# QuakeMigrate/QuakeMigrate

Measured on AMD Instinct MI355X. Metric: grid-nodes x time-samples stacked /sec (detect sweep), higher is better.
Workload: dtype f64

## Files before the change

### __graft_entry__.py

```python

import pathlib
import shutil
import subprocess
import sys
import sysconfig

ROOT = pathlib.Path(__file__).resolve().parent
CSRC = ROOT / "quakemigrate_amd" / "csrc"
if str(ROOT) not in sys.path:
    sys.path.insert(0, str(ROOT))

HIPCC_FLAGS = ["--offload-arch=gfx950", "-O3", "-std=c++17", "-fPIC"]
OBJ = CSRC / "build"


def _run(cmd, **kw):
    print("+", " ".join(str(c) for c in cmd), flush=True)
    subprocess.check_call([str(c) for c in cmd], **kw)


def _stale(target, sources):
    if not target.exists():
        return True
    t = target.stat().st_mtime
    return any(pathlib.Path(s).stat().st_mtime > t for s in sources)


def build_engine(force=False):
    import concurrent.futures
    import os

    for generator, include in (("gen_ring_asm.py", "qm_ring_asm.inc"), ("gen_shift_asm.py", "qm_shift_asm.inc")):
        gen = subprocess.check_output([sys.executable, str(CSRC / generator)], text=True)
        inc = CSRC / include
        if not inc.exists() or inc.read_text() != gen:
            inc.write_text(gen)
    srcs = sorted(CSRC.glob("qm_*.hip")) + [CSRC / "qm_stalta.cpp"]
    headers = sorted(CSRC.glob("*.hpp")) + sorted(CSRC.glob("*.inc")) + [ROOT / "include" / "qmhip.h"]
    link_inputs = [CSRC / "qmhip.map"]
    hipcc = shutil.which("hipcc") or "/opt/rocm/bin/hipcc"
    OBJ.mkdir(exist_ok=True)
    objs = [OBJ / (src.name + ".o") for src in srcs]
    lib = CSRC / "libqmhip.so"
    todo = []
    if force or _stale(lib, srcs + headers):
        todo = [(src, obj) for src, obj in zip(srcs, objs) if force or _stale(obj, [src] + headers)]
    if todo:
        todo.sort(key=lambda so: ("pair" not in so[0].name, "exact" not in so[0].name))
        with concurrent.futures.ThreadPoolExecutor(max(1, min(len(todo), os.cpu_count() or 1))) as pool:
            asm_unit = ["-Wno-inline-asm", "-Wno-pass-failed", "-save-temps=obj", "-Wno-unused-command-line-argument"]
            quiet = {"qm_launch_shift.hip": asm_unit, "qm_launch_shift_sets.hip": asm_unit}
            list(pool.map(lambda so: _run([hipcc, *HIPCC_FLAGS, *quiet.get(so[0].name, []), "-c", so[0],
                                           "-o", so[1]]), todo))
        if any(src.name.startswith("qm_launch_shift") for src, _ in todo):
            check_row_block_registers()
    if force or todo or _stale(lib, srcs + headers + link_inputs):
        _run([hipcc, "--offload-arch=gfx950", "-shared", "-fPIC", f"-Wl,--version-script={CSRC / 'qmhip.map'}",
              "-o", lib, *objs])
    alias = CSRC / ("qmlib" + sysconfig.get_config_var("EXT_SUFFIX"))
    if force or _stale(alias, [lib]):
        shutil.copyfile(lib, alias)
    return lib


def check_row_block_registers():
    sys.path.insert(0, str(CSRC))
    try:
        import check_shift_isa
    finally:
        sys.path.pop(0)
    found = sorted(OBJ.glob("qm_launch_shift-*gfx950*.s"))
    if not found:
        raise RuntimeError("build: the ISA of qm_launch_shift.hip was not kept (-save-temps=obj): the "
                           "row-block kernels' register convention cannot be checked")
    n = check_shift_isa.check_all(found[-1].read_text(), (CSRC / "qm_shift_asm.inc").read_text())
    print(f"build: row-block kernels keep to their registers ({n} compiler instructions checked)")
    for tmp in OBJ.glob("qm_launch_shift*"):
        if tmp.suffix in (".bc", ".hipi", ".hipfb", ".out", ".o", ".txt") and not tmp.name.endswith(".hip.o"):
            tmp.unlink()
        elif tmp.suffix == ".s" and "gfx950" not in tmp.name:
            tmp.unlink()


def build_oracle():
    _run(["make", "-C", ROOT / "oracle", "libqm_oracle.so"])
    _run(["make", "-C", ROOT / "oracle", "ref"])


def build():
    build_engine()
    build_oracle()
    import quakemigrate_amd
    from quakemigrate_amd import core

    print("build ok:", CSRC / "libqmhip.so")


def smoke():
    import numpy as np

    from oracle import qm_oracle
    from quakemigrate_amd import synth
    from quakemigrate_amd.core import lib

    if lib.qmlib.qm_device_count() < 1:
        raise RuntimeError("smoke(): no HIP device visible")
    case = synth.make_case("C2", step=0, grid=(26, 25, 14), n_samples=700)
    a, b, c = lib.migrate_and_find_max(case.onsets, case.traveltimes, case.fsmp,
                                       case.lsmp, case.available)
    ra, rb, rc = qm_oracle.detect(case.onsets, case.traveltimes, case.fsmp,
                                  case.lsmp, case.available, threads=4)
    assert np.array_equal(c, rc), "argmax mismatch vs oracle"
    np.testing.assert_allclose(a, ra, rtol=1e-6)
    np.testing.assert_allclose(b, rb, rtol=1e-6)
    print("smoke ok: fused detect == oracle on", case.grid, "x", case.n_samples,
          "samples; max rel err", float(np.max(np.abs(a - ra) / ra)))


if __name__ == "__main__":
    build()
    if len(sys.argv) > 1 and sys.argv[1] == "smoke":
        smoke()
```

### quakemigrate_amd/csrc/qm_shift.hpp

```cpp
#pragma once

#include "qm_kernels.hpp"

namespace qm {

struct ShiftStageNext {
    const void *meta;
    int rows;
    int first_row, stride;
    const void *src;
    unsigned row_bytes;
    unsigned lds;
    unsigned lane32;
};

#ifndef QM_SHIFT_ASM_INC
#define QM_SHIFT_ASM_INC "qm_shift_asm.inc"
#endif
#include QM_SHIFT_ASM_INC

constexpr int kShiftWaves = 4;
constexpr int kShiftWaves8 = 8;
constexpr int kShiftWaves3 = 12;
constexpr int kShiftKT = 256;
constexpr int kShiftWideKT = kWave * kShiftWideSpl;
constexpr int kShiftLdsBytes = 2 * kShiftPlane;
constexpr int kShiftStateBytes = 5 * kShiftStateChunk;
constexpr int kShiftLdsBytes3 = 2 * kShiftPlane3 + kShiftWaves3 * kShiftStateBytes;
static_assert(kShiftLdsBytes3 <= 160 * 1024, "the 12-wave workgroup's LDS exceeds a CU's");
constexpr int kShiftLdsBytes8 = 2 * kShiftPlane8;
static_assert(kShiftLdsBytes8 <= 160 * 1024, "the 8-wave workgroup's LDS exceeds a CU's");
__host__ __device__ constexpr int shift_plane(int nw) {
    return nw == kShiftWaves3 ? kShiftPlane3 : nw == kShiftWaves8 ? kShiftPlane8 : kShiftPlane;
}
__host__ __device__ constexpr int shift_lds_bytes(int nw) {
    return nw == kShiftWaves3 ? kShiftLdsBytes3 : nw == kShiftWaves8 ? kShiftLdsBytes8 : kShiftLdsBytes;
}
constexpr int kShiftMaxRows = 64;
constexpr int kShiftHalfBytes = 80 * 1024;
static_assert(2 * kShiftPlane <= kShiftHalfBytes, "a half holds both planes");
static_assert(QM_EXP2_DEGREE_SUM == 8 && QM_EXP2_DEGREE_VOLUME == kShiftVolumeDegree,
              "the generated loops carry the degree-8 (detect) 2^f and the stored values' degree");

__host__ __device__ constexpr bool shift_packed(bool blocks) { return blocks ? kShiftPackedBlocks : kShiftPackedGroups; }
__host__ __device__ constexpr int shift_rec_bytes(bool blocks) { return shift_packed(blocks) ? 32 : 64; }
constexpr int kShiftRec = shift_rec_bytes(false);
constexpr int kShiftRecBlocks = shift_rec_bytes(true);
__host__ __device__ constexpr int shift_rec_hdr(bool packed) { return packed ? 2 : 8; }
__host__ __device__ constexpr int shift_rec_base(bool packed) { return packed ? 4 : 10; }

__host__ __device__ __forceinline__ int shift_groups_per_brick(const GridDesc &g) {
    return (g.bx / 2) * (g.by / 2) * (g.bz / 2);
}
__host__ __device__ __forceinline__ int64_t shift_recs_per_wave(const GridDesc &g, int rows2, int nw) {
    return (int64_t)((shift_groups_per_brick(g) + nw - 1) / nw) * rows2 + 2;
}
__host__ __device__ __forceinline__ int64_t shift_run_record(int64_t b, int w, int k, int nw, int nblk,
                                                             int64_t rpw) {
    return ((b * nw + w) * nblk + k) * rpw;
}

struct ShiftArgs {
    StackArgs a;
    const int4 *smeta;
    const int32_t *stotal;
    const int32_t *sfit;
    const char *stream;
    int rows2;
    int nw;
    int lazy;
    int nblk;
    int sb;
    int stage_slots;
    int stage_reach;
    const int4 *wmeta;
    const int32_t *wtotal;
    const char *wstream;
};

constexpr int kShiftLazyGroups = 160;

constexpr int kShiftDetect = 0;
constexpr int kShiftVolume = 1;
constexpr int kShiftMarginal = 2;

struct LaunchShape;
const char *shift_unit_defines();
hipError_t launch_shift_detect(const ShiftArgs &a, const LaunchShape &s);
hipError_t launch_shift_volume(const ShiftArgs &a, const LaunchShape &s);
hipError_t launch_shift_marginal(const ShiftArgs &a, const LaunchShape &s);
hipError_t launch_shift_marginal8(const ShiftArgs &a, const LaunchShape &s);
hipError_t launch_shift_detect3(const ShiftArgs &a, const LaunchShape &s);
hipError_t launch_shift_detect8(const ShiftArgs &a, const LaunchShape &s);
hipError_t launch_shift_volume8(const ShiftArgs &a, const LaunchShape &s);
hipError_t launch_shift_rows8(const ShiftArgs &a, const LaunchShape &s);
hipError_t launch_shift_rows2(const ShiftArgs &a, const LaunchShape &s);
hipError_t launch_shift_rows2_volume(const ShiftArgs &a, const LaunchShape &s);
hipError_t launch_shift_rows4(const ShiftArgs &a, const LaunchShape &s);
hipError_t launch_shift_rows4_volume(const ShiftArgs &a, const LaunchShape &s);
hipError_t launch_shift_wide_rows(const ShiftArgs &a, const LaunchShape &s);
hipError_t launch_shift_detect_sets(const ShiftArgs &a, const LaunchShape &s);
hipError_t launch_shift_detect8_sets(const ShiftArgs &a, const LaunchShape &s);

__device__ __forceinline__ void shift_group_box(const GridDesc &g, int b, int &x0, int &y0, int &z0,
                                                int &vx, int &vy, int &vz, int &cx, int &cy,
                                                int &cz) {
    brick_extents(g, b, x0, y0, z0, vx, vy, vz);
    cx = (vx + 1) / 2; cy = (vy + 1) / 2; cz = (vz + 1) / 2;
}

__device__ __forceinline__ unsigned shift_group_delays(const GridDesc &g, const int32_t *lut, int x0,
                                                       int y0, int z0, int vx, int vy, int vz,
                                                       int gx, int gy, int gz, int r, int lo,
                                                       int (&d)[8]) {
    unsigned mask = 0;
#pragma unroll
    for (int n = 0; n < 8; ++n) {
        const int lx = 2 * gx + (n >> 2), ly = 2 * gy + ((n >> 1) & 1), lz = 2 * gz + (n & 1);
        if (lx < vx && ly < vy && lz < vz) {
            const int64_t node = ((int64_t)(x0 + lx) * g.ny + (y0 + ly)) * g.nz + (z0 + lz);
            int t = lut[node * g.n_rows + r];
            t = t < 0 ? 0 : t;
            d[n] = t - lo;
            mask |= 1u << n;
        } else {
            d[n] = d[0];
        }
    }
    return mask;
}

__device__ __forceinline__ void shift_window(const int (&d)[8], int wide, int &e0, int &nq) {
    int dmin = d[0], dmax = d[0];
#pragma unroll
    for (int n = 1; n < 8; ++n) {
        dmin = d[n] < dmin ? d[n] : dmin;
        dmax = d[n] > dmax ? d[n] : dmax;
    }
    e0 = wide ? dmin & ~1 : dmin & ~3;
    nq = (dmax - e0 + (wide ? kShiftWideSpl : 4) + 3) / 4;
    nq = nq < 2 ? 2 : nq;
}
__host__ __device__ constexpr int shift_lane_step(int wide) { return wide ? kShiftWideSpl : 4; }
__host__ __device__ constexpr int shift_slots_touched(int wide, int e0, int fetched) {
    return (e0 + shift_lane_step(wide) * (kWave - 1) + 4 * fetched + 3) / 4;
}
__host__ __device__ constexpr int shift_nq_min(int wide) { return wide ? kShiftNqMinWide : kShiftNqMin; }
__host__ __device__ constexpr int shift_zero_slots(int wide) {
    return wide ? shift_slots_touched(1, 0, kShiftNqMinWide) : kWave + kShiftNqMin;
}

#ifdef QM_TU_TABLES
__global__ __launch_bounds__(256) void shift_need_kernel(GridDesc g, const int32_t *__restrict__ lut,
                                                         const int4 *__restrict__ meta_raw,
                                                         int4 *__restrict__ smeta,
                                                         int32_t *__restrict__ stotal,
                                                         int32_t *__restrict__ sfit,
                                                         unsigned long long *__restrict__ tally,
                                                         int plane_bytes, int nblk, int sb, int wide) {
    __shared__ int need[kShiftMaxRows];
    __shared__ int overflow;
    const int vb = blockIdx.x, b = vb / nblk, r0 = (vb % nblk) * sb;
    const int S = g.n_rows - r0 < sb ? g.n_rows - r0 : sb;
    int x0, y0, z0, vx, vy, vz, cx, cy, cz;
    shift_group_box(g, b, x0, y0, z0, vx, vy, vz, cx, cy, cz);
    for (int r = threadIdx.x; r < S; r += blockDim.x) need[r] = 0;
    if (threadIdx.x == 0) overflow = 0;
    __syncthreads();
    const int nvg = cx * cy * cz;
    unsigned quads = 0;
    for (int i = threadIdx.x; i < nvg * S; i += blockDim.x) {
        const int j = i / S, r = i % S;
        const int gz = j % cz, gy = (j / cz) % cy, gx = j / (cz * cy);
        int d[8], e0, nq;
        shift_group_delays(g, lut, x0, y0, z0, vx, vy, vz, gx, gy, gz, r0 + r,
                           meta_raw[(int64_t)b * g.n_rows + r0 + r].x, d);
        shift_window(d, wide, e0, nq);
        if (nq > kShiftNqMax) atomicOr(&overflow, 1);
        const int fetched = nq > shift_nq_min(wide) ? nq : shift_nq_min(wide);
        quads += (unsigned)fetched;
        atomicMax(&need[r], shift_slots_touched(wide, e0, fetched));
    }
    atomicAdd(&tally[0], (unsigned long long)quads);
    __syncthreads();
    if (threadIdx.x == 0) {
        atomicAdd(&tally[1], (unsigned long long)nvg * S);
        int run = 0;
        for (int r = 0; r < S; ++r) {
            const int4 raw = meta_raw[(int64_t)b * g.n_rows + r0 + r];
            smeta[(int64_t)vb * sb + r] = make_int4(raw.x, raw.y, run, need[r]);
            run += need[r];
            atomicMax(&tally[2], (unsigned long long)need[r]);
            const int reach = raw.x + 4 * need[r];
            atomicMax(&tally[3], (unsigned long long)(reach > 0 ? reach : 0));
        }
        stotal[vb] = run;
        const int zero_row = (S & 1) ? shift_zero_slots(wide) : 0;
        sfit[vb] = (!overflow && (int64_t)(run + zero_row) * 16 <= plane_bytes) ? 1 : 0;
    }
}

__global__ __launch_bounds__(256) void shift_stream_kernel(GridDesc g, const int32_t *__restrict__ lut,
                                                           const int4 *__restrict__ smeta,
                                                           const int32_t *__restrict__ stotal,
                                                           const int32_t *__restrict__ sfit, int rows2max,
                                                           int nw, int nblk, int sb, int packed, int wide,
                                                           uint32_t *__restrict__ stream) {
    extern __shared__ uint2 hdr[];
    const int vb = blockIdx.x, b = vb / nblk, k = vb % nblk, r0 = k * sb;
    const int S = g.n_rows - r0 < sb ? g.n_rows - r0 : sb;
    const int rows2 = S + (S & 1);
    if (!sfit[b]) return;
    int x0, y0, z0, vx, vy, vz, cx, cy, cz;
    shift_group_box(g, b, x0, y0, z0, vx, vy, vz, cx, cy, cz);
    const int nvg = cx * cy * cz;
    const int64_t rpw = shift_recs_per_wave(g, rows2max, nw);
    auto record = [&](int w, int64_t i) {
        return stream + (shift_run_record(b, w, k, nw, nblk, rpw) + i) * (packed ? 8 : 16);
    };
    for (int i = threadIdx.x; i < nvg * rows2; i += blockDim.x) {
        const int j = i / rows2, r = i % rows2;
        const int w = j % nw, pos = j / nw;
        uint32_t *rec = record(w, 1 + (int64_t)pos * rows2 + r);
        if (r >= S) {
            for (int n = 0; n < (packed ? 2 : 8); ++n) rec[n] = 0;
            hdr[j * rows2 + r] = make_uint2(16u * (unsigned)stotal[vb], 2u);
            continue;
        }
        const int gz = j % cz, gy = (j / cz) % cy, gx = j / (cz * cy);
        const int4 m = smeta[(int64_t)vb * sb + r];
        int d[8], e0, nq;
        const unsigned mask = shift_group_delays(g, lut, x0, y0, z0, vx, vy, vz, gx, gy, gz, r0 + r, m.x, d);
        shift_window(d, wide, e0, nq);
        if (packed) {
            uint32_t lo = 0, hi = 0;
            for (int n = 0; n < 4; ++n) {
                lo |= (2u * (unsigned)(d[n] - e0)) << (8 * n);
                hi |= (2u * (unsigned)(d[4 + n] - e0)) << (8 * n);
            }
            rec[0] = lo;
            rec[1] = hi;
        } else {
            for (int n = 0; n < 8; ++n) rec[n] = 2u * (unsigned)(d[n] - e0);
        }
        hdr[j * rows2 + r] = make_uint2(16u * (unsigned)m.z + 4u * (unsigned)e0, (unsigned)nq);
        if (r == 0) {
            rec[shift_rec_base(packed)] = (uint32_t)(((int64_t)(x0 + 2 * gx) * g.ny + (y0 + 2 * gy)) * g.nz + (z0 + 2 * gz));
            rec[shift_rec_base(packed) + 1] = mask;
        }
    }
    __syncthreads();
    for (int i = threadIdx.x; i < nvg * rows2 + nw; i += blockDim.x) {
        if (i >= nvg * rows2) {
            const int w = i - nvg * rows2;
            if (w < nvg) {
                const uint2 h = hdr[w * rows2];
                uint32_t *rec = record(w, 0);
                rec[shift_rec_hdr(packed)] = h.x;
                rec[shift_rec_hdr(packed) + 1] = h.y;
            }
            continue;
        }
        const int j = i / rows2, r = i % rows2;
        const int w = j % nw, pos = j / nw;
        uint32_t *rec = record(w, 1 + (int64_t)pos * rows2 + r);
        uint2 h = make_uint2(0u, 2u);
        if (r + 1 < rows2) h = hdr[j * rows2 + r + 1];
        else if (j + nw < nvg) h = hdr[(j + nw) * rows2];
        rec[shift_rec_hdr(packed)] = h.x;
        rec[shift_rec_hdr(packed) + 1] = h.y;
    }
}
#endif

#ifdef QM_SHIFT_TU
template <int NW, int RB = (NW == 12 ? 3 : 8), int U = 6, bool CONTIG = false, int KT = kShiftKT>
__device__ __forceinline__ void stage_shift_windows(const ShiftArgs &s, double *win, int vb, int row0,
                                                    int S, int sb, int wave, int lane, int t_first) {
    const StackArgs &a = s.a;
    constexpr bool kWide = KT == kShiftWideKT;
    const int4 *const smeta = kWide ? s.wmeta : s.smeta;
    const int32_t *const stotal = kWide ? s.wtotal : s.stotal;
    constexpr int kPlane = shift_plane(NW);
    auto where = [&](int z, int u) {
        if constexpr (CONTIG) return 4 * z + u;
        else return ((u & 2) ? kPlane / 8 : 0) + 2 * (z + (u >> 2)) + (u & 1);
    };
    for (int r0 = wave; r0 < S; r0 += NW * RB) {
        double v[RB][U];
        int4 m[RB];
#pragma unroll
        for (int k = 0; k < RB; ++k) {
            const int r = r0 + k * NW;
            m[k] = r < S ? smeta[(int64_t)vb * sb + r] : make_int4(0, 0, 0, 0);
            const int len = m[k].y + KT;
            const int first = m[k].x + a.fsmp + a.sample0 + t_first;
            const int room = a.T - first;
            const double *src = a.onsets + (int64_t)(r < S ? row0 + r : 0) * a.T + first;
#pragma unroll
            for (int i = 0; i < U; ++i) {
                const int u = kWave * i + lane;
                v[k][i] = (r < S && u < len && u < room) ? src[u] : 0.0;
            }
        }
#pragma unroll
        for (int k = 0; k < RB; ++k) {
            const int total = 4 * m[k].w;
#pragma unroll
            for (int i = 0; i < U; ++i) {
                const int u = kWave * i + lane;
                if (u < total) win[where(m[k].z, u)] = v[k][i];
            }
            if (total > kWave * U) {
                const int r = r0 + k * NW;
                const int len = m[k].y + KT;
                const int first = m[k].x + a.fsmp + a.sample0 + t_first;
                const int room = a.T - first;
                const double *src = a.onsets + (int64_t)(row0 + r) * a.T + first;
                for (int u = kWave * U + lane; u < total; u += kWave)
                    win[where(m[k].z, u)] = (u < len && u < room) ? src[u] : 0.0;
            }
        }
    }
    if ((S & 1) && wave == 0) {
        const int z = stotal[vb];
        for (int u = lane; u < 4 * shift_zero_slots(kWide); u += kWave) win[where(z, u)] = 0.0;
    }
}

template <int NW>
__device__ __forceinline__ void stage_shift_wide(const ShiftArgs &s, double *win, int vb, int S, int wave,
                                                 int lane, int t_first, int row0 = 0, int sb = 0) {
    const StackArgs &a = s.a;
    using int4s = int __attribute__((ext_vector_type(4)));
    const int4s *meta = reinterpret_cast<const int4s *>(s.wmeta + (int64_t)vb * (sb ? sb : S));
    const unsigned lds_base = (unsigned)(uintptr_t)((lds_f64 *)win);
    const unsigned lane16 = (unsigned)lane * 16u;
    for (int r = wave; r < S; r += NW) {
        const int4s m = meta[__builtin_amdgcn_readfirstlane(r)];
        const int first = __builtin_amdgcn_readfirstlane(m.x) + a.fsmp + a.sample0 + t_first;
        const int total = 4 * __builtin_amdgcn_readfirstlane(m.w);
        const int z4 = 4 * __builtin_amdgcn_readfirstlane(m.z);
        const int room = a.T - first;
        const double *src = a.onsets + (int64_t)(row0 + r) * a.T + first;
        if (room >= total) {
            const unsigned long long sp = (unsigned long long)src;
            const double *usrc = (const double *)(((unsigned long long)(unsigned)__builtin_amdgcn_readfirstlane((int)(sp >> 32)) << 32) |
                                                  (unsigned)__builtin_amdgcn_readfirstlane((int)sp));
            for (int c = 0; c < total; c += 2 * kWave) {
                const int pairs = (total - c) / 2 < kWave ? (total - c) / 2 : kWave;
                unsigned long long saved;
                asm volatile("s_mov_b64 %[sv], exec\n\t"
                             "s_lshr_b64 exec, -1, %[sh]\n\t"
                             "s_mov_b32 m0, %[ma]\n\t"
                             "s_nop 0\n\t"
                             "global_load_lds_dwordx4 %[vo], %[src]\n\t"
                             "s_mov_b64 exec, %[sv]"
                             : [sv] "=&s"(saved)
                             : [sh] "s"(__builtin_amdgcn_readfirstlane(kWave - pairs)),
                               [ma] "s"(__builtin_amdgcn_readfirstlane((int)(lds_base + 8u * (unsigned)(z4 + c)))),
                               [vo] "v"(lane16), [src] "s"(usrc + c)
                             : "memory", "m0");
            }
        } else {
            const int len = __builtin_amdgcn_readfirstlane(m.y) + kShiftWideKT;
            for (int u = lane; u < total; u += kWave) win[z4 + u] = (u < len && u < room) ? src[u] : 0.0;
        }
    }
    if ((S & 1) && wave == 0) {
        const int z4 = 4 * s.wtotal[vb];
        for (int u = lane; u < 4 * shift_zero_slots(1); u += kWave) win[z4 + u] = 0.0;
    }
}

struct ShiftWork {
    int tile, group, spl;
    int t_own;
    int t_first;
    bool run;
};
__device__ __forceinline__ ShiftWork shift_work(const StackArgs &a) {
    ShiftWork w;
    stack_tile_group(a, w.tile, w.group);
    w.run = w.group < a.ngroups && !(a.run_if != nullptr && *a.run_if == 0);
    if (w.tile < a.wide_tiles) {
        w.spl = kShiftWideSpl;
        w.t_own = w.tile * kShiftWideKT;
        w.t_first = w.t_own + kShiftWideKT > a.n_chunk ? a.n_chunk - kShiftWideKT : w.t_own;
        return w;
    }
    w.spl = (a.tail_spl > 0 && w.tile == a.ntiles - 1) ? a.tail_spl : 4;
    w.t_own = a.wide_tiles * kShiftWideKT + (w.tile - a.wide_tiles) * kShiftKT;
    w.t_first = (w.spl == 4 && w.t_own + kShiftKT > a.n_chunk && a.n_chunk >= kShiftKT)
                    ? a.n_chunk - kShiftKT : w.t_own;
    return w;
}
template <int J>
__device__ __forceinline__ void shift_reset(double (&vmax)[J], double (&vsum)[J], int (&vidx)[J]) {
#pragma unroll
    for (int k = 0; k < J; ++k) {
        vmax[k] = -__builtin_inf();
        vsum[k] = 0.0;
        vidx[k] = INT32_MAX;
    }
}

template <int NW, int J = 4>
__device__ __forceinline__ void shift_publish(const StackArgs &a, double *win, const double (&vmax)[J],
                                              const double (&vsum)[J], const int (&vidx)[J], int wave,
                                              int lane, int group, int t_first, int t_own = 0) {
    constexpr int KT = kWave * J;
    double *smax = win, *ssum = win + NW * KT;
    int *sidx = reinterpret_cast<int *>(win + 2 * NW * KT);
#pragma unroll
    for (int k = 0; k < J; ++k) {
        const int o = wave * KT + J * lane + k;
        smax[o] = vmax[k];
        ssum[o] = vsum[k];
        sidx[o] = vidx[k];
    }
    __syncthreads();
    const int k = threadIdx.x;
    if (k >= KT) return;
    double best = smax[k], total = ssum[k];
    int bi = sidx[k];
    for (int w = 1; w < NW; ++w) {
        const double v = smax[w * KT + k];
        const int i = sidx[w * KT + k];
        total += ssum[w * KT + k];
        if (better(v, i, best, bi)) {
            best = v;
            bi = i;
        }
    }
    const int t = t_first + k;
    if (t < a.n_chunk && t >= t_own) {
        const int64_t o = (int64_t)(a.set0 + group) * (a.part_stride ? a.part_stride : a.n_chunk) + t;
        a.part_max[o] = best;
        a.part_idx[o] = bi == INT32_MAX ? kNoIndex : (int64_t)bi;
        a.part_sum[o] = total;
    }
}

template <int MODE, int NW, int J, bool WIDE_LAZY = false, int SETS = 0>
__device__ __forceinline__ void shift_tile(const ShiftArgs &s, double *win, const ShiftWork &work,
                                           int lane, int wave) {
    constexpr bool kLdsState = NW == kShiftWaves3;
    constexpr bool kWide = J == kShiftWideSpl;
    constexpr bool kTail = J != 4;
    static_assert(!(kTail && kLdsState), "the 12-wave shape has no tail flavours");
    static_assert(!kWide || (MODE == kShiftDetect && NW == kShiftWaves8), "wide tiles: fused detect, 8 waves");
    static_assert(!SETS || (MODE == kShiftDetect && !kLdsState), "brick maxima: fused detect, 4 or 8 waves");
    static_assert(SETS != 2 || kWide, "brick maxima from the generated loop: wide tiles");
    const StackArgs &a = s.a;
    const GridDesc &g = a.g;
    const int tile = work.tile, group = work.group, t_first = work.t_first;
    const unsigned lds_base = (unsigned)(uintptr_t)((lds_f64 *)win);
    const unsigned lane_addr = lds_base + (unsigned)lane * (kTail ? 8u * J : 16u);
    const int seam = work.t_own - t_first;
    const unsigned long long store_lanes = ~0ull << (seam / 4);
    unsigned long long slot_lanes[J];
    double weight[J];
#pragma unroll
    for (int k = 0; k < J; ++k) {
        const int t = t_first + J * lane + k;
        slot_lanes[k] = __builtin_amdgcn_ballot_w64(t < a.n_chunk);
        weight[k] = (t >= work.t_own && t >= a.m0 && t < a.m1 && t < a.n_chunk) ? 1.0 : 0.0;
    }
    const int lane_node = 4 * ((lane >> 2) & 1) + 2 * (lane & 1) + ((lane >> 1) & 1);
    const unsigned node_off = 8u * (unsigned)((lane_node & 4 ? g.ny * g.nz : 0) + (lane_node & 2 ? g.nz : 0) +
                                             (lane_node & 1));
    const unsigned lane_x16 = 4u * (unsigned)(lane ^ 16), lane_x32 = 4u * (unsigned)(lane ^ 32);
    (void)store_lanes; (void)slot_lanes; (void)weight; (void)node_off; (void)lane_x16; (void)lane_x32;

    double vmax[J], vsum[J];
    int vidx[J];
    shift_reset<J>(vmax, vsum, vidx);
    double *state = win + (2 * shift_plane(NW) + wave * kShiftStateBytes) / 8 + 2 * lane;
    const unsigned state_addr = (unsigned)(uintptr_t)((lds_f64 *)state);
    if constexpr (kLdsState) {
#pragma unroll
        for (int k = 0; k < 4; ++k) {
            state[(k / 2) * (kShiftStateChunk / 8) + (k & 1)] = vmax[k];
            state[(2 + k / 2) * (kShiftStateChunk / 8) + (k & 1)] = vsum[k];
            reinterpret_cast<int *>(state + 4 * (kShiftStateChunk / 8))[k] = vidx[k];
        }
    }
    (void)state_addr;
    constexpr int D = MODE == kShiftVolume ? Exp2Degree<true>::value
                      : MODE == kShiftMarginal ? kShiftMarginalDegree : Exp2Degree<false>::value;
    double c[D + 1];
#pragma unroll
    for (int i = 0; i <= D; ++i) c[i] = exp2_coeff<D>(i);

    const int64_t rpw = shift_recs_per_wave(g, s.rows2, NW);
    const int npairs = s.rows2 / 2, nz = g.nz, nynz = g.ny * g.nz;
    double *const marg_tile = a.marginal + (int64_t)tile * a.n_nodes;
    double *const vol_tile = a.volume + t_first;
    const unsigned vol_stride_bytes = (unsigned)(a.vol_stride * 8);
    (void)marg_tile; (void)vol_tile; (void)vol_stride_bytes;
    double wmax[J];
    int widx[J];
    (void)wmax; (void)widx;
    const int64_t brow_stride = a.part_stride ? a.part_stride : a.n_chunk;
    if constexpr (SETS == 1) {
#pragma unroll
        for (int k = 0; k < J; ++k) {
            wmax[k] = -__builtin_inf();
            widx[k] = INT32_MAX;
        }
    }
    auto brick_row = [&](int b) {
        constexpr int KT = kWave * J;
#pragma unroll
        for (int k = 0; k < J; ++k) win[wave * KT + J * lane + k] = vmax[k];
        __syncthreads();
        const int j = threadIdx.x;
        if (j < KT && t_first + j < a.n_chunk && t_first + j >= work.t_own) {
            double best = win[j];
            for (int w = 1; w < NW; ++w) best = win[w * KT + j] > best ? win[w * KT + j] : best;
            a.brick_max[(int64_t)b * brow_stride + t_first + j] = best;
        }
#pragma unroll
        for (int k = 0; k < J; ++k) {
            if (better(vmax[k], vidx[k], wmax[k], widx[k])) {
                wmax[k] = vmax[k];
                widx[k] = vidx[k];
            }
            vmax[k] = -__builtin_inf();
            vidx[k] = INT32_MAX;
        }
    };
    int prev = -1;
    for (int b = group; b < g.nbricks; b += a.ngroups) {
        if constexpr (SETS == 1) {
            if (prev >= 0) {
                __syncthreads();
                brick_row(prev);
            }
            prev = b;
        }
        if (!s.sfit[b]) continue;
#ifdef QM_SHIFT_EXP_NOSTAGE
        if (b == group) {
            if constexpr (kWide) {
                stage_shift_wide<NW>(s, win, b, g.n_rows, wave, lane, t_first);
                asm volatile("s_waitcnt vmcnt(0)" ::: "memory");
            } else {
                stage_shift_windows<NW>(s, win, b, 0, g.n_rows, g.n_rows, wave, lane, t_first);
            }
            __syncthreads();
        }
#else
        __syncthreads();
        if constexpr (kWide) {
            stage_shift_wide<NW>(s, win, b, g.n_rows, wave, lane, t_first);
            asm volatile("s_waitcnt vmcnt(0)" ::: "memory");
        } else {
            stage_shift_windows<NW, (NW == 12 ? 3 : 8), 6, kTail, kWave * J>(s, win, b, 0, g.n_rows, g.n_rows, wave,
                                                                             lane, t_first);
        }
        __syncthreads();
#endif
        int x0, y0, z0, vx, vy, vz, cx, cy, cz;
        shift_group_box(g, b, x0, y0, z0, vx, vy, vz, cx, cy, cz);
        const int nvg = cx * cy * cz;
        const int mine = (nvg - wave + NW - 1) / NW;
        if (mine <= 0) continue;
        const char *const stream = kWide ? s.wstream : s.stream;
        const char *run = stream + shift_run_record(b, wave, 0, NW, 1, rpw) * kShiftRec;
        int nb = b + a.ngroups;
        while (nb < g.nbricks && !s.sfit[nb]) nb += a.ngroups;
        const char *next_run = stream + shift_run_record(nb < g.nbricks ? nb : b, wave, 0, NW, 1, rpw) * kShiftRec;
        const unsigned next_off = (unsigned)lane * 64u;
        const void *next_meta = s.smeta + (int64_t)(nb < g.nbricks ? nb : b) * g.n_rows;
        (void)next_meta;
        const unsigned lane_addr_b = lane_addr + (unsigned)kShiftPlane8;
#ifdef QM_SHIFT_DEPHASE
        if (NW == kShiftWaves8 && (wave & 4)) __builtin_amdgcn_s_sleep(QM_SHIFT_DEPHASE);
#endif
        (void)lane_addr_b; (void)next_run; (void)next_off;
#define QM_TAIL_CALL(JJ)                                                                              \
        if constexpr (MODE == kShiftMarginal)                                                         \
            shift_tail##JJ##_marginal(vmax, vsum, vidx, run, mine, next_run, next_off, next_meta, npairs, lane_addr, nz, nynz,       \
                                      a.z_scale, c, marg_tile, weight, node_off, lane_x16, lane_x32); \
        else if constexpr (MODE == kShiftVolume)                                                      \
            shift_tail##JJ##_volume(vmax, vsum, vidx, run, mine, next_run, next_off, next_meta, npairs, lane_addr, nz, nynz,         \
                                    a.z_scale, c, vol_tile, vol_stride_bytes, (unsigned)lane * (8u * JJ), \
                                    slot_lanes);                                                      \
        else                                                                                          \
            shift_tail##JJ##_detect(vmax, vsum, vidx, run, mine, next_run, next_off, next_meta, npairs, lane_addr, nz, nynz,         \
                                    a.z_scale, c)
        const char *const brow = reinterpret_cast<const char *>(a.brick_max + (int64_t)b * brow_stride + t_first) -
                                 lds_base;
        (void)brow;
        if constexpr (kWide && WIDE_LAZY && SETS == 2)
            shift_wide_detect_bmax_lazy(vmax, vsum, vidx, run, mine, next_run, next_off, next_meta, npairs, lane_addr,
                                        brow, nz, nynz, a.z_scale, c);
        else if constexpr (kWide && SETS == 2)
            shift_wide_detect_bmax(vmax, vsum, vidx, run, mine, next_run, next_off, next_meta, npairs, lane_addr,
                                   brow, nz, nynz, a.z_scale, c);
        else if constexpr (kWide && WIDE_LAZY)
            shift_wide_detect_lazy(vmax, vsum, vidx, run, mine, next_run, next_off, next_meta, npairs, lane_addr, nz, nynz,
                                   a.z_scale, c);
        else if constexpr (kWide)
            shift_wide_detect(vmax, vsum, vidx, run, mine, next_run, next_off, next_meta, npairs, lane_addr, nz, nynz,
                              a.z_scale, c);
        else if constexpr (J == 1) { QM_TAIL_CALL(1); }
        else if constexpr (J == 2) { QM_TAIL_CALL(2); }
        else if constexpr (J == 3) { QM_TAIL_CALL(3); }
#undef QM_TAIL_CALL
        else if constexpr (kLdsState)
            shift_groups_detect3(run, mine, next_run, next_off, next_meta, npairs, lane_addr, state_addr, nz, nynz, a.z_scale, c);
        else if constexpr (NW == kShiftWaves8 && MODE == kShiftMarginal)
            shift_groups_marginal8(vmax, vsum, vidx, run, mine, next_run, next_off, next_meta, npairs, lane_addr, lane_addr_b, nz, nynz,
                                   a.z_scale, c, marg_tile, weight, node_off, lane_x16, lane_x32);
        else if constexpr (MODE == kShiftMarginal)
            shift_groups_marginal(vmax, vsum, vidx, run, mine, next_run, next_off, next_meta, npairs, lane_addr, nz, nynz, a.z_scale, c,
                                  marg_tile, weight, node_off, lane_x16, lane_x32);
        else if constexpr (NW == kShiftWaves8 && MODE == kShiftVolume)
            shift_groups_volume8(vmax, vsum, vidx, run, mine, next_run, next_off, next_meta, npairs, lane_addr, lane_addr_b, nz, nynz,
                                 a.z_scale, c, vol_tile, vol_stride_bytes, (unsigned)lane * 32u, store_lanes);
        else if constexpr (NW == kShiftWaves8) {
            if (s.lazy && SETS != 1)
                shift_groups_detect8_lazy(vmax, vsum, vidx, run, mine, next_run, next_off, next_meta, npairs, lane_addr, lane_addr_b, nz,
                                          nynz, a.z_scale, c);
            else
                shift_groups_detect8(vmax, vsum, vidx, run, mine, next_run, next_off, next_meta, npairs, lane_addr, lane_addr_b, nz, nynz,
                                     a.z_scale, c);
        }
        else if constexpr (MODE == kShiftVolume)
            shift_groups_volume(vmax, vsum, vidx, run, mine, next_run, next_off, next_meta, npairs, lane_addr, nz, nynz, a.z_scale, c,
                                vol_tile, vol_stride_bytes, (unsigned)lane * 32u, store_lanes);
        else if (s.lazy && SETS != 1)
            shift_groups_detect_lazy(vmax, vsum, vidx, run, mine, next_run, next_off, next_meta, npairs, lane_addr, nz, nynz, a.z_scale, c);
        else
            shift_groups_detect(vmax, vsum, vidx, run, mine, next_run, next_off, next_meta, npairs, lane_addr, nz, nynz, a.z_scale, c);
    }
    if (!a.want_scan) return;
    if constexpr (kLdsState) {
#pragma unroll
        for (int k = 0; k < 4; ++k) {
            vmax[k] = state[(k / 2) * (kShiftStateChunk / 8) + (k & 1)];
            vsum[k] = state[(2 + k / 2) * (kShiftStateChunk / 8) + (k & 1)];
            vidx[k] = reinterpret_cast<int *>(state + 4 * (kShiftStateChunk / 8))[k];
        }
    }
    __syncthreads();
    if constexpr (SETS == 1) {
        brick_row(prev);
#pragma unroll
        for (int k = 0; k < J; ++k) {
            vmax[k] = wmax[k];
            vidx[k] = widx[k];
        }
        __syncthreads();
    }
    shift_publish<NW, J>(a, win, vmax, vsum, vidx, wave, lane, group, t_first, work.t_own);
}

template <int MODE, int NW, bool SETS>
__device__ __forceinline__ void stack_shift_body(ShiftArgs &s, double *win) {
    static_assert(NW == kShiftWaves || NW == kShiftWaves8 || (NW == kShiftWaves3 && MODE == kShiftDetect),
                  "workgroup shapes: 4 or 8 waves, or 12 (detect only)");
    const int lane = threadIdx.x & (kWave - 1);
    const int wave = __builtin_amdgcn_readfirstlane(threadIdx.x >> 6);
    if constexpr (MODE == kShiftDetect) s.a = step_view(s.a);
    const ShiftWork work = shift_work(s.a);
    if (!work.run) return;
    if constexpr (MODE == kShiftDetect && NW == kShiftWaves8) {
        if (work.spl == kShiftWideSpl) {
            if constexpr (SETS) {
                if (s.lazy) return shift_tile<MODE, NW, kShiftWideSpl, true, 2>(s, win, work, lane, wave);
                return shift_tile<MODE, NW, kShiftWideSpl, false, 2>(s, win, work, lane, wave);
            }
            if (s.lazy) return shift_tile<MODE, NW, kShiftWideSpl, true, 0>(s, win, work, lane, wave);
            return shift_tile<MODE, NW, kShiftWideSpl, false, 0>(s, win, work, lane, wave);
        }
    }
    if constexpr (NW != kShiftWaves3) {
        if (work.spl == 3) return shift_tile<MODE, NW, 3, false, SETS ? 1 : 0>(s, win, work, lane, wave);
        if (work.spl == 2) return shift_tile<MODE, NW, 2, false, SETS ? 1 : 0>(s, win, work, lane, wave);
        if (work.spl == 1) return shift_tile<MODE, NW, 1, false, SETS ? 1 : 0>(s, win, work, lane, wave);
    }
    shift_tile<MODE, NW, 4, false, SETS ? 1 : 0>(s, win, work, lane, wave);
}

template <int MODE, int NW>
__global__ __launch_bounds__(NW * kWave, NW == kShiftWaves3 ? 3 : 2) void stack_shift_kernel(ShiftArgs s) {
    extern __shared__ __attribute__((aligned(16))) double win[];
    stack_shift_body<MODE, NW, false>(s, win);
}
template <int NW>
__global__ __launch_bounds__(NW * kWave, 2) void stack_shift_bricks_kernel(ShiftArgs s) {
    extern __shared__ __attribute__((aligned(16))) double win[];
    stack_shift_body<kShiftDetect, NW, true>(s, win);
}

__device__ __forceinline__ const void *shift_meta_ahead(const ShiftArgs &s, const GridDesc &g, int b, int nb,
                                                        int k, const int4 *smeta = nullptr) {
    if (smeta == nullptr) smeta = s.smeta;
    int pb = b, pk = k + 2;
    if (pk >= s.nblk) {
        pb = nb;
        pk -= s.nblk;
        if (pk >= s.nblk) {
            pb = nb + s.a.ngroups;
            pk = 0;
        }
    }
    if (pb >= g.nbricks) pb = b, pk = 0;
    return smeta + ((int64_t)pb * s.nblk + pk) * s.sb;
}

#ifndef QM_ROWS_RB
#define QM_ROWS_RB 3
#define QM_ROWS_U 5
#endif
template <int NW>
__global__ __attribute__((amdgpu_flat_work_group_size(NW * kWave, NW * kWave), amdgpu_waves_per_eu(6, 6)))
void stack_shift_rows_kernel(ShiftArgs s) {
    static_assert(NW == kShiftWaves8, "row blocks: the 8-wave workgroup");
    extern __shared__ __attribute__((aligned(16))) double win[];
    const StackArgs &a = s.a;
    const GridDesc &g = a.g;
    const int lane = threadIdx.x & (kWave - 1);
    const int wave = __builtin_amdgcn_readfirstlane(threadIdx.x >> 6);
    const ShiftWork work = shift_work(a);
    if (!work.run) return;
    const int tile = work.tile, group = work.group, t_first = work.t_first;
    const unsigned lane_addr = (unsigned)(uintptr_t)((lds_f64 *)win) + (unsigned)lane * 16u;

    double vmax[4], vsum[4];
    int vidx[4];
    shift_reset(vmax, vsum, vidx);
    constexpr int D = Exp2Degree<false>::value;
    double c[D + 1];
#pragma unroll
    for (int i = 0; i <= D; ++i) c[i] = exp2_coeff<D>(i);

    const int rows2max = s.sb + (s.sb & 1);
    const int64_t rpw = shift_recs_per_wave(g, rows2max, NW);
    for (int b = group; b < g.nbricks; b += a.ngroups) {
        if (!s.sfit[b]) continue;
        int x0, y0, z0, vx, vy, vz, cx, cy, cz;
        shift_group_box(g, b, x0, y0, z0, vx, vy, vz, cx, cy, cz);
        const bool mine = wave < cx * cy * cz;
        int nb = b + a.ngroups;
        while (nb < g.nbricks && !s.sfit[nb]) nb += a.ngroups;
        const char *next_run = s.stream + shift_run_record(nb < g.nbricks ? nb : b, wave, 0, NW, s.nblk, rpw) * kShiftRecBlocks;
        for (int k = 0; k < s.nblk; ++k) {
            const void *next_meta = shift_meta_ahead(s, g, b, nb, k);
            const int row0 = k * s.sb;
            const int rows = g.n_rows - row0 < s.sb ? g.n_rows - row0 : s.sb;
            __syncthreads();
            stage_shift_windows<NW, QM_ROWS_RB, QM_ROWS_U>(s, win, b * s.nblk + k, row0, rows, s.sb, wave,
                                                           lane, t_first);
            __syncthreads();
            if (mine) {
                const char *run = s.stream + shift_run_record(b, wave, k, NW, s.nblk, rpw) * kShiftRecBlocks;
                const unsigned flags = (unsigned)__builtin_amdgcn_readfirstlane(
                    (int)((k == 0 ? 1u : 0u) | (k == s.nblk - 1 ? 2u : 0u)));
                shift_group_rows8(vmax, vsum, vidx, run, flags, next_run, (unsigned)lane * 64u, next_meta,
                                  (rows + 1) / 2, lane_addr, lane_addr + (unsigned)kShiftPlane8, g.nz,
                                  g.ny * g.nz, a.z_scale, c);
            }
        }
    }
    if (!a.want_scan) return;
    __syncthreads();
    shift_publish<NW>(a, win, vmax, vsum, vidx, wave, lane, group, t_first);
}


__device__ __forceinline__ void stage_shift_zero_row(const ShiftArgs &s, double *half, int vb, int S, int wave,
                                                     int lane) {
    if ((S & 1) && wave == 0) {
        const int z = s.stotal[vb];
        for (int u = lane; u < 4 * (64 + kShiftNqMin); u += kWave)
            half[((u & 2) ? kShiftPlane / 8 : 0) + 2 * (z + (u >> 2)) + (u & 1)] = 0.0;
    }
}

template <int NW>
__device__ __forceinline__ void stage_shift_block_direct(const ShiftArgs &s, double *half, int vb,
                                                         int row0, int S, int wave, int lane,
                                                         int t_first) {
    const StackArgs &a = s.a;
    using lds_ptr = __attribute__((address_space(3))) void *;
    using glb_ptr = const __attribute__((address_space(1))) void *;
    constexpr int R = (34 + NW - 1) / NW;
    using int4s = int __attribute__((ext_vector_type(4)));
    int4s ms[R];
    if constexpr (NW == kShiftWaves8) {
        static_assert(R == 5, "five metadata loads per wavefront and block");
        const int4 *base = s.smeta + (int64_t)vb * s.sb;
        unsigned off[R];
#pragma unroll
        for (int j = 0; j < R; ++j) {
            const int r = wave + j * NW;
            off[j] = (unsigned)__builtin_amdgcn_readfirstlane((r < S ? r : 0) * 16);
        }
        asm volatile("s_load_dwordx4 %0, %5, %6\n\ts_load_dwordx4 %1, %5, %7\n\ts_load_dwordx4 %2, %5, %8\n\t"
                     "s_load_dwordx4 %3, %5, %9\n\ts_load_dwordx4 %4, %5, %10\n\ts_waitcnt lgkmcnt(0)"
                     : "=&s"(ms[0]), "=&s"(ms[1]), "=&s"(ms[2]), "=&s"(ms[3]), "=&s"(ms[4])
                     : "s"(base), "s"(off[0]), "s"(off[1]), "s"(off[2]), "s"(off[3]), "s"(off[4])
                     : "memory");
    } else {
        const int4s *base = reinterpret_cast<const int4s *>(s.smeta + (int64_t)vb * s.sb);
#pragma unroll
        for (int j = 0; j < R; ++j) {
            const int r = wave + j * NW;
            ms[j] = base[__builtin_amdgcn_readfirstlane(r < S ? r : 0)];
        }
    }
    int4 meta[R];
#pragma unroll
    for (int j = 0; j < R; ++j) meta[j] = make_int4(ms[j].x, ms[j].y, ms[j].z, ms[j].w);
#pragma unroll
    for (int j = 0; j < R; ++j) {
        const int r = wave + j * NW;
        if (r >= S) break;
        const int4 m = meta[j];
        const int first = m.x + a.fsmp + a.sample0 + t_first;
        const int room = a.T - first;
        const double *src = a.onsets + (int64_t)(row0 + r) * a.T + first;
#ifndef QM_ROWS_STAGE_SLOW
        if (room >= 4 * m.w) {
            const unsigned la = (unsigned)__builtin_amdgcn_readfirstlane(
                (int)((unsigned)(uintptr_t)((lds_f64 *)half) + 16u * (unsigned)m.z));
            const unsigned long long sp = (unsigned long long)src;
            src = (const double *)(((unsigned long long)(unsigned)__builtin_amdgcn_readfirstlane((int)(sp >> 32)) << 32) |
                                   (unsigned)__builtin_amdgcn_readfirstlane((int)sp));
            const int slots = __builtin_amdgcn_readfirstlane(m.w);
            const unsigned lane32 = (unsigned)lane * 32u;
            for (int c = 0; c < slots; c += kWave) {
                const int n = slots - c < kWave ? slots - c : kWave;
                unsigned long long saved;
                asm volatile("s_mov_b64 %[sv], exec\n\t"
                             "s_lshr_b64 exec, -1, %[sh]\n\t"
                             "s_mov_b32 m0, %[ma]\n\t"
                             "s_nop 0\n\t"
                             "global_load_lds_dwordx4 %[vo], %[src]\n\t"
                             "s_mov_b32 m0, %[mb]\n\t"
                             "s_nop 0\n\t"
                             "global_load_lds_dwordx4 %[vo], %[src] offset:16\n\t"
                             "s_mov_b64 exec, %[sv]"
                             : [sv] "=&s"(saved)
                             : [sh] "s"(kWave - n), [ma] "s"(la + 16u * (unsigned)c),
                               [mb] "s"(la + 16u * (unsigned)c + (unsigned)kShiftPlane - 16u), [vo] "v"(lane32),
                               [src] "s"(src + 4 * c)
                             : "memory", "m0");
            }
            continue;
        }
#endif
        for (int c = 0; c * kWave < m.w; ++c) {
            const int slot = c * kWave + lane;
            if (slot < m.w) {
                const int u = 4 * slot;
                double *la = half + 2 * (m.z + c * kWave);
                double *lb = la + kShiftPlane / 8;
                if (room - u >= 2)
                    __builtin_amdgcn_global_load_lds((glb_ptr)(src + u), (lds_ptr)(lds_f64 *)la, 16, 0, 0);
                else if (room - u == 1)
                    la[2 * lane] = src[u];
                if (room - u >= 4)
                    __builtin_amdgcn_global_load_lds((glb_ptr)(src + u + 2), (lds_ptr)(lds_f64 *)lb, 16, 0, 0);
                else if (room - u == 3)
                    lb[2 * lane] = src[u + 2];
            }
        }
    }
    stage_shift_zero_row(s, half, vb, S, wave, lane);
}

template <bool VOLUME, int NW>
__global__ __attribute__((amdgpu_flat_work_group_size(NW * kWave, NW * kWave), amdgpu_waves_per_eu(6, 6)))
void stack_shift_rows2_kernel(ShiftArgs s) {
    static_assert(NW == kShiftWaves8, "row blocks: the 8-wave workgroup");
    extern __shared__ __attribute__((aligned(16))) double win[];
    const StackArgs &a = s.a;
    const GridDesc &g = a.g;
    const int lane = threadIdx.x & (kWave - 1);
    const int wave = __builtin_amdgcn_readfirstlane(threadIdx.x >> 6);
    const ShiftWork work = shift_work(a);
    if (!work.run) return;
    const int tile = work.tile, group = work.group, t_first = work.t_first;
    const unsigned lane_addr = (unsigned)(uintptr_t)((lds_f64 *)win) + (unsigned)lane * 16u;
    const int seam = tile * kShiftKT - t_first;
    const unsigned long long store_lanes = ~0ull << (seam / 4);

    double vmax[4], vsum[4];
    int vidx[4];
    shift_reset(vmax, vsum, vidx);
    constexpr int D = Exp2Degree<VOLUME>::value;
    double c[D + 1];
#pragma unroll
    for (int i = 0; i <= D; ++i) c[i] = exp2_coeff<D>(i);

    const int rows2max = s.sb + (s.sb & 1);
    const int64_t rpw = shift_recs_per_wave(g, rows2max, NW);
    auto rows_of = [&](int k) { return g.n_rows - k * s.sb < s.sb ? g.n_rows - k * s.sb : s.sb; };
    const int tile_room = a.T - (a.fsmp + a.sample0 + t_first);
    const bool in_loop = kShiftStageInLoop && s.stage_slots <= 127 && tile_room >= s.stage_reach &&
                         a.T < (1 << 28);
    int b = group;
    while (b < g.nbricks && !s.sfit[b]) b += a.ngroups;
    int cur = 0;
    if (b < g.nbricks)
        stage_shift_block_direct<NW>(s, win, b * s.nblk, 0, rows_of(0), wave, lane, t_first);
    asm volatile("s_waitcnt vmcnt(0)" ::: "memory");
    __syncthreads();
    while (b < g.nbricks) {
        int nb = b + a.ngroups;
        while (nb < g.nbricks && !s.sfit[nb]) nb += a.ngroups;
        int x0, y0, z0, vx, vy, vz, cx, cy, cz;
        shift_group_box(g, b, x0, y0, z0, vx, vy, vz, cx, cy, cz);
        const bool mine = wave < cx * cy * cz;
        const char *next_run =
            s.stream + shift_run_record(nb < g.nbricks ? nb : b, wave, 0, NW, s.nblk, rpw) * kShiftRecBlocks;
        for (int k = 0; k < s.nblk; ++k) {
            const void *next_meta = shift_meta_ahead(s, g, b, nb, k);
            double *idle = win + (cur ^ 1) * (kShiftHalfBytes / 8);
            const bool follows = k + 1 < s.nblk || nb < g.nbricks;
            const int vbn = k + 1 < s.nblk ? b * s.nblk + k + 1 : nb * s.nblk;
            const int kn = k + 1 < s.nblk ? k + 1 : 0;
            ShiftStageNext stage{};
            stage.meta = s.smeta;
#ifndef QM_ROWS_EXP_NOSTAGE
            if (follows && in_loop && mine) {
                stage_shift_zero_row(s, idle, vbn, rows_of(kn), wave, lane);
                stage.meta = s.smeta + (int64_t)vbn * s.sb;
                stage.rows = rows_of(kn);
                stage.first_row = wave;
                stage.stride = NW;
                stage.src = a.onsets + (int64_t)kn * s.sb * a.T + a.fsmp + a.sample0 + t_first;
                stage.row_bytes = (unsigned)a.T * 8u;
                stage.lds = (unsigned)(uintptr_t)((lds_f64 *)idle);
                stage.lane32 = (unsigned)lane * 32u;
// ... 202 lines not shown
```

Before: 603.1 billion.

## Add a separate row loop for node groups cut by the grid edge

Generates a second form of each fused-detect assembly loop. Node groups that are whole take the original unguarded loop, and groups cut by the grid's edge take a loop that tests a node mask and skips the adds for absent nodes. Every detect call site now uses the new _cut variants. The aim is to spend fewer adds on padded edge nodes, or to drop per-node guards from full groups, in exchange for larger code, extra branching and more generated assembly to keep correct.

```diff
diff --git a/__graft_entry__.py b/__graft_entry__.py
--- a/__graft_entry__.py
+++ b/__graft_entry__.py
@@ -30,7 +30,8 @@
     import concurrent.futures
     import os
 
-    for generator, include in (("gen_ring_asm.py", "qm_ring_asm.inc"), ("gen_shift_asm.py", "qm_shift_asm.inc")):
+    for generator, include in (("gen_ring_asm.py", "qm_ring_asm.inc"), ("gen_shift_asm.py", "qm_shift_asm.inc"),
+                               ("gen_shift_cut_asm.py", "qm_shift_cut_asm.inc")):
         gen = subprocess.check_output([sys.executable, str(CSRC / generator)], text=True)
         inc = CSRC / include
         if not inc.exists() or inc.read_text() != gen:
diff --git a/quakemigrate_amd/csrc/gen_shift_cut_asm.py b/quakemigrate_amd/csrc/gen_shift_cut_asm.py
--- /dev/null
+++ b/quakemigrate_amd/csrc/gen_shift_cut_asm.py
@@ -0,0 +1,128 @@
+#!/usr/bin/env python3
+import contextlib
+
+import gen_shift_asm as G
+
+FLAVOURS = (
+    (8, False, False, "shift_groups_detect", 4, False, False),
+    (8, False, True, "shift_groups_detect_lazy", 4, False, False),
+    (8, True, False, "shift_groups_detect8", 4, False, False),
+    (8, True, True, "shift_groups_detect8_lazy", 4, False, False),
+    (8, False, False, "shift_tail1_detect", 1, True, False),
+    (8, False, False, "shift_tail2_detect", 2, True, False),
+    (8, False, False, "shift_tail3_detect", 3, True, False),
+    (8, False, False, "shift_wide_detect", 6, True, False),
+    (8, False, True, "shift_wide_detect_lazy", 6, True, False),
+    (8, False, False, "shift_wide_detect_bmax", 6, True, True),
+    (8, False, True, "shift_wide_detect_bmax_lazy", 6, True, True),
+)
+
+
+def cut_node_adds(e, p, g, first):
+    assert G.PACKED and G.PACKED_SHIFT64 and not G.BLOCK
+    rec = G.BUF[p]
+    if g in (1, 2, 3):
+        e(f"s_lshr_b64 {G.s2(rec)}, {G.s2(rec)}, 8")
+    absent = e.label("ab")
+    e(f"s_bitcmp1_b32 s{G.SMASK}, {g}")
+    e(f"s_cbranch_scc0 {absent}")
+    e(f"s_set_gpr_idx_on s{rec + g // 4}, 1")
+    for k in range(G.SPL):
+        a = G.v2(G.ACC + G.AS * g + 2 * k)
+        e(f"v_add_f64 {a}, {G.v2(G.WIN[p] + 2 * k)}, {'0' if first else a}")
+    e(f"{absent}:")
+
+
+@contextlib.contextmanager
+def cut_nodes():
+    whole, G.node_adds = G.node_adds, cut_node_adds
+    try:
+        yield
+    finally:
+        G.node_adds = whole
+
+
+def cut_rows(e, cut, epi, group):
+    end, pair = e.label("ce"), e.label("cp")
+    e("s_waitcnt lgkmcnt(0)")
+    e(f"s_cselect_b32 s{G.SPAIRS}, s{G.BUF[0] + G.R_BASE + 1}, 0")
+    e(f"s_cmpk_eq_u32 s{G.SPAIRS}, 0xff")
+    e(f"s_cbranch_scc1 {group}")
+    e("s_cmp_eq_u32 %[ng], 0")
+    e(f"s_cbranch_scc1 {end}")
+    e(f"{cut}:")
+    with cut_nodes():
+        G.row_iter(e, 0, True)
+        G.row_iter(e, 1, False)
+        e(f"s_sub_u32 s{G.SPAIRS}, %[npairs], 2")
+        e(f"s_cbranch_scc1 {epi}")
+        e(f"{pair}:")
+        G.row_iter(e, 0, False)
+        G.row_iter(e, 1, False)
+    e(f"s_sub_u32 s{G.SPAIRS}, s{G.SPAIRS}, 1")
+    e(f"s_cbranch_scc0 {pair}")
+    e(f"s_branch {epi}")
+    e(f"{end}:")
+
+
+def body(degree, volume):
+    assert not (volume or G.BLOCK or G.LDS_STATE) and G.NEXT_RUN and not G.NEXT_META
+    e = G.Emitter()
+    e(f"v_mov_b32 v{G.VC}, %[clo]")
+    e(f"v_mov_b32 v{G.VC + 1}, %[chi]")
+    e(f"s_mov_b32 s{G.STAB}, %[tablo]")
+    e(f"s_mov_b32 s{G.STAB + 1}, %[tabhi]")
+    e(f"s_load_dwordx{G.NBUF} s[{G.BUF[1]}:{G.BUF[1] + G.NBUF - 1}], {G.s2(G.STAB)}, 0")
+    e(f"s_load_dwordx{G.NBUF} s[{G.BUF[0]}:{G.BUF[0] + G.NBUF - 1}], {G.s2(G.STAB)}, {G.REC}")
+    e(f"s_mov_b32 s{G.SOFF}, {G.REC}")
+    e(f"s_mov_b32 s{G.SNEGINF}, 0")
+    e(f"s_mov_b32 s{G.SNEGINF + 1}, 0xfff00000")
+    e(f"s_mov_b32 s{G.SMAGIC}, 0")
+    e(f"s_mov_b32 s{G.SMAGIC + 1}, 0x43380000")
+    e(f"v_mov_b32 v{G.VZERO}, 0")
+    if G.LAZY:
+        e(f"v_mov_b32 v{G.VMAG}, 0")
+        e(f"v_mov_b32 v{G.VMAG + 1}, 0x43380000")
+    e(f"s_add_u32 s{G.SPF}, s{G.STAB}, {G.PF_AHEAD * G.REC}")
+    e(f"s_addc_u32 s{G.SPF + 1}, s{G.STAB + 1}, 0")
+    e("s_waitcnt lgkmcnt(0)")
+    G.issue_window(e, 0, G.BUF[1] + G.R_HDR)
+    group, pair, nopair = e.label("grp"), e.label("pair"), e.label("np")
+    e(f"global_load_dword v{G.VPF}, %[nxoff], %[nxrun]")
+    cut, epi = e.label("cut"), e.label("epi")
+    e(f"s_cmpk_lg_u32 s{G.BUF[0] + G.R_BASE + 1}, 0xff")
+    e(f"s_cbranch_scc1 {cut}")
+    G.STAGING = False
+    e(f"{group}:")
+    G.row_iter(e, 0, True)
+    G.row_iter(e, 1, False)
+    e(f"s_sub_u32 s{G.SPAIRS}, %[npairs], 2")
+    e(f"s_cbranch_scc1 {nopair}")
+    e(f"{pair}:")
+    G.row_iter(e, 0, False)
+    G.row_iter(e, 1, False)
+    e(f"s_sub_u32 s{G.SPAIRS}, s{G.SPAIRS}, 1")
+    e(f"s_cbranch_scc0 {pair}")
+    e(f"{nopair}:")
+    e(f"{epi}:")
+    G.epilogue(e, degree, volume)
+    e("s_sub_u32 %[ng], %[ng], 1")
+    e("s_cmp_lg_u32 %[ng], 0")
+    cut_rows(e, cut, epi, group)
+    e("s_waitcnt vmcnt(0) lgkmcnt(0)")
+    return e.lines
+
+
+def main():
+    print("// GENERATED by gen_shift_cut_asm.py -- do not edit.  The fused-detect loops of qm_shift_asm.inc with a second")
+    print("// form of the row loop for node groups cut by the grid's edge; see that file.")
+    whole, G.body = G.body, body
+    try:
+        for degree, far, lazy, name, spl, contig, bmax in FLAVOURS:
+            G.emit(degree, False, False, far, lazy, False, name + "_cut", spl, contig, bmax=bmax)
+    finally:
+        G.body = whole
+
+
+if __name__ == "__main__":
+    main()
diff --git a/quakemigrate_amd/csrc/qm_shift.hpp b/quakemigrate_amd/csrc/qm_shift.hpp
--- a/quakemigrate_amd/csrc/qm_shift.hpp
+++ b/quakemigrate_amd/csrc/qm_shift.hpp
@@ -18,6 +18,10 @@
 #define QM_SHIFT_ASM_INC "qm_shift_asm.inc"
 #endif
 #include QM_SHIFT_ASM_INC
+#ifndef QM_SHIFT_CUT_ASM_INC
+#define QM_SHIFT_CUT_ASM_INC "qm_shift_cut_asm.inc"
+#endif
+#include QM_SHIFT_CUT_ASM_INC
 
 constexpr int kShiftWaves = 4;
 constexpr int kShiftWaves8 = 8;
@@ -589,22 +593,22 @@
                                     a.z_scale, c, vol_tile, vol_stride_bytes, (unsigned)lane * (8u * JJ), \
                                     slot_lanes);                                                      \
         else                                                                                          \
-            shift_tail##JJ##_detect(vmax, vsum, vidx, run, mine, next_run, next_off, next_meta, npairs, lane_addr, nz, nynz,         \
+            shift_tail##JJ##_detect_cut(vmax, vsum, vidx, run, mine, next_run, next_off, next_meta, npairs, lane_addr, nz, nynz,         \
                                     a.z_scale, c)
         const char *const brow = reinterpret_cast<const char *>(a.brick_max + (int64_t)b * brow_stride + t_first) -
                                  lds_base;
         (void)brow;
         if constexpr (kWide && WIDE_LAZY && SETS == 2)
-            shift_wide_detect_bmax_lazy(vmax, vsum, vidx, run, mine, next_run, next_off, next_meta, npairs, lane_addr,
+            shift_wide_detect_bmax_lazy_cut(vmax, vsum, vidx, run, mine, next_run, next_off, next_meta, npairs, lane_addr,
                                         brow, nz, nynz, a.z_scale, c);
         else if constexpr (kWide && SETS == 2)
-            shift_wide_detect_bmax(vmax, vsum, vidx, run, mine, next_run, next_off, next_meta, npairs, lane_addr,
+            shift_wide_detect_bmax_cut(vmax, vsum, vidx, run, mine, next_run, next_off, next_meta, npairs, lane_addr,
                                    brow, nz, nynz, a.z_scale, c);
         else if constexpr (kWide && WIDE_LAZY)
-            shift_wide_detect_lazy(vmax, vsum, vidx, run, mine, next_run, next_off, next_meta, npairs, lane_addr, nz, nynz,
+            shift_wide_detect_lazy_cut(vmax, vsum, vidx, run, mine, next_run, next_off, next_meta, npairs, lane_addr, nz, nynz,
                                    a.z_scale, c);
         else if constexpr (kWide)
-            shift_wide_detect(vmax, vsum, vidx, run, mine, next_run, next_off, next_meta, npairs, lane_addr, nz, nynz,
+            shift_wide_detect_cut(vmax, vsum, vidx, run, mine, next_run, next_off, next_meta, npairs, lane_addr, nz, nynz,
                               a.z_scale, c);
         else if constexpr (J == 1) { QM_TAIL_CALL(1); }
         else if constexpr (J == 2) { QM_TAIL_CALL(2); }
@@ -623,19 +627,19 @@
                                  a.z_scale, c, vol_tile, vol_stride_bytes, (unsigned)lane * 32u, store_lanes);
         else if constexpr (NW == kShiftWaves8) {
             if (s.lazy && SETS != 1)
-                shift_groups_detect8_lazy(vmax, vsum, vidx, run, mine, next_run, next_off, next_meta, npairs, lane_addr, lane_addr_b, nz,
+                shift_groups_detect8_lazy_cut(vmax, vsum, vidx, run, mine, next_run, next_off, next_meta, npairs, lane_addr, lane_addr_b, nz,
                                           nynz, a.z_scale, c);
             else
-                shift_groups_detect8(vmax, vsum, vidx, run, mine, next_run, next_off, next_meta, npairs, lane_addr, lane_addr_b, nz, nynz,
+                shift_groups_detect8_cut(vmax, vsum, vidx, run, mine, next_run, next_off, next_meta, npairs, lane_addr, lane_addr_b, nz, nynz,
                                      a.z_scale, c);
         }
         else if constexpr (MODE == kShiftVolume)
             shift_groups_volume(vmax, vsum, vidx, run, mine, next_run, next_off, next_meta, npairs, lane_addr, nz, nynz, a.z_scale, c,
                                 vol_tile, vol_stride_bytes, (unsigned)lane * 32u, store_lanes);
         else if (s.lazy && SETS != 1)
-            shift_groups_detect_lazy(vmax, vsum, vidx, run, mine, next_run, next_off, next_meta, npairs, lane_addr, nz, nynz, a.z_scale, c);
+            shift_groups_detect_lazy_cut(vmax, vsum, vidx, run, mine, next_run, next_off, next_meta, npairs, lane_addr, nz, nynz, a.z_scale, c);
         else
-            shift_groups_detect(vmax, vsum, vidx, run, mine, next_run, next_off, next_meta, npairs, lane_addr, nz, nynz, a.z_scale, c);
+            shift_groups_detect_cut(vmax, vsum, vidx, run, mine, next_run, next_off, next_meta, npairs, lane_addr, nz, nynz, a.z_scale, c);
     }
     if (!a.want_scan) return;
     if constexpr (kLdsState) {
```

After: 605.1 billion (median of 6 runs). Within noise of the previous version (+0.3%).
